# ProteusMRIgHIFU/BabelBrain

Measured on AMD Instinct MI355X. Metric: Mvoxel-steps/sec, 512^3 skull FDTD per device (achieved HBM GB/s in roofline), higher is better.
Workload: dtype f32

## Files before the change

babelbrain_amd/csrc/bfd_api.hip:

```cpp
#include "bfd_internal.h"

#include <math.h>
#include <stdio.h>
#include <string.h>

#include <algorithm>
#include <array>
#include <thread>
#include <hipcub/hipcub.hpp>

static thread_local std::string g_err;
void bfd_set_error(const std::string &s) { g_err = s; }

namespace {

struct HostTables {
    std::vector<float> t;
    float c1, k2;
    double cmax;
};

void fit_sls(double rho, double c, double alpha, double q, double omega, bool exact, double &MR, double &tau)
{
    if (c <= 0.0) { MR = 0.0; tau = 0.0; return; }
// ... 469 lines not shown
        BFD_FAIL(-2, "bfd_create: h, dt, freq must be > 0 and 0 < reflectionLimit < 1");
    int ndev = 0;
    if (hipGetDeviceCount(&ndev) != hipSuccess || ndev <= 0)
        BFD_FAIL(-3, "bfd_create: no HIP device available (this engine has no CPU fallback)");
    if (cfg->device < 0 || cfg->device >= ndev) BFD_FAIL(-3, "bfd_create: device ordinal out of range");
    BFD_HIP(hipSetDevice(cfg->device));

    bfd_sim *s = new bfd_sim();
    s->cfg = *cfg;
    s->step = 0; s->devBytes = 0; s->haveMaterials = s->haveMap = false; s->tilesReady = false;
    s->nSrcVox = 0; s->srcLin = s->srcRow = nullptr; s->srcW[0] = s->srcW[1] = s->srcW[2] = nullptr; s->pulseT = nullptr;
    s->nSources = s->lengthSource = 0;
    s->pulseHost = nullptr; s->tileSteps = s->nTiles = 0;
    s->srcK = 0; s->srcWeights = s->srcSignals = nullptr;
    for (int b = 0; b < 2; b++) { s->tileDev[b] = s->tilePinned[b] = nullptr; s->tileLoaded[b] = s->tilePacked[b] = -1; s->evTile[b] = nullptr; s->evTileUsed[b] = false; for (int q = 0; q < 2; q++) { s->evRead[b][q] = nullptr; s->evReadUsed[b][q] = false; } }
    s->sensEnt = nullptr; s->sensEntValid = false; s->sensIsBox = false; memset(s->sensBox, 0, sizeof s->sensBox);
    s->actBase = nullptr; s->actBytes = 0; s->actReady = false;
    s->nSensors = 0; s->sensLin = nullptr; s->sensOut = nullptr; s->dftAcc = nullptr; s->dftPk = nullptr; s->dftBin = 0;
    s->acc = s->pk = nullptr; s->timing = s->perKernel = false;
    s->pairEnv = true; s->pendingAcc = s->pairDone = false; s->pairedLaunches = 0;
    if (const char *ev = getenv("BFD_PAIR_ACC")) s->pairEnv = atoi(ev) != 0;
    s->advEnv = true; s->midStep = false; s->tiles.advVz = false;
    if (const char *ev = getenv("BFD_ADV_VZ")) s->advEnv = atoi(ev) != 0;
    s->tables = nullptr; s->profiles = nullptr; s->cmax = 0;
    memset(s->algBytes, 0, sizeof s->algBytes); s->tiles.ktimer = nullptr;
    if (hipStreamCreateWithFlags(&s->stream, hipStreamNonBlocking) != hipSuccess) { delete s; BFD_FAIL(-10, "hipStreamCreate failed"); }
    s->ownStream = true;
    if (hipEventCreate(&s->evBegin) != hipSuccess) { hipStreamDestroy(s->stream); delete s; BFD_FAIL(-10, "hipEventCreate failed"); }
    if (hipEventCreate(&s->evEnd) != hipSuccess) { hipEventDestroy(s->evBegin); hipStreamDestroy(s->stream); delete s; BFD_FAIL(-10, "hipEventCreate failed"); }

    bfd_dev &d = s->d;
    memset(&d, 0, sizeof d);
    d.N1 = cfg->N1; d.N2 = cfg->N2; d.N3 = cfg->N3; d.k0 = cfg->k0; d.nk = cfg->nk;
    d.ND = cfg->NDelta; d.P = P; d.plane = cfg->N1 * cfg->N2;
    s->nloc = (size_t)d.plane * d.nk;
    s->nalloc = (size_t)d.plane * (d.nk + 4);
    bfd_placement_cache_evict_other_sizes(cfg->device, s->nalloc * sizeof(float));

    int rc = 0;
    float **fp[15] = {&d.Vx, &d.Vy, &d.Vz, &d.Sxx, &d.Syy, &d.Szz, &d.Sxy, &d.Sxz, &d.Syz,
                      &d.Rxx, &d.Ryy, &d.Rzz, &d.Rxy, &d.Rxz, &d.Ryz};
    for (int a = 0; a < 15 && !rc; a++) {
        rc = dev_alloc(s, &s->stateBase[a], s->nalloc);
        if (!rc) *fp[a] = s->stateBase[a] + 2 * (size_t)d.plane;
    }
    if (!rc) rc = dev_alloc(s, &s->matBase, s->nalloc);
// ... 626 lines not shown
    const bool pairAcc = pair_engine(s, quiet_runs_wanted(s), T.nFluid);
    for (size_t r = 0; r < all.size(); r++) {
        const int4 &run = all[r];
        const int bx = run.x % tx, by = run.x / tx, kb = run.y & 0xFFFF, ke = run.y >> 16, f = run.z;
        const int xa = bx * 64, xb = std::min(xa + 64, N1), ya = by * 8, yb = std::min(ya + 8, N2);
        const double cells = (double)(xb - xa) * (yb - ya) * (ke - kb);
        const double inner = overlap(xa, xb, ND, N1 - ND) * overlap(ya, yb, ND, N2 - ND) * overlap(k0g + kb, k0g + ke, ND, N3 - ND);
        const bool fusedRun = r >= (size_t)(T.nFluid + T.nSolid);
        if (fusedRun) {
            const double fc = 64.0 * bfd_fused_rows() * (ke - kb);
            const double b = 32.0 + ((f & 2) ? 8.0 : 0.0) + ((f & 4) ? 0.0 : 2.0);
            B[0][BFD_K_FUSED] += b * fc; B[1][BFD_K_FUSED] += b * fc + 8.0 * fc;
        } else if (r < (size_t)T.nFluid) {
            const bool lossy = f & 2, uni = f & 4, single = (f & 16) != 0;
            double bs = 12.0 + 8.0 + (lossy ? 8.0 : 0.0) + (uni ? 0.0 : 2.0);
            if (!single) bs += 8.0 + (lossy ? 8.0 : 0.0);
            const double bv = 4.0 + 24.0 + (uni ? 0.0 : 2.0);
            for (int a = 0; a < 2; a++) { B[a][BFD_K_STRESS_FLUID] += bs * cells; B[a][BFD_K_VELOCITY_FLUID] += bv * cells; }
            if (pairAcc) B[1][BFD_K_STRESS_FLUID] += 4.0 * inner; else B[1][BFD_K_VELOCITY_FLUID] += 8.0 * inner;
            if (f & BFD_RUN_ADV_VZ) {
                const double advCells = (double)(xb - xa) * (yb - ya) * std::max(0, ke - kb - 3);
                for (int a = 0; a < 2; a++) { B[a][BFD_K_STRESS_FLUID] += 4.0 * advCells; B[a][BFD_K_VELOCITY_FLUID] -= 8.0 * advCells; }
            }
        } else if (s->cfg.kernelVariant == 2) {
            for (int a = 0; a < 2; a++) { B[a][BFD_K_STRESS_SOLID] += 110.0 * cells; B[a][BFD_K_VELOCITY_SOLID] += 50.0 * cells + (a ? 8.0 * inner : 0.0); }
        } else {
            for (int a = 0; a < 2; a++) B[a][BFD_K_VELOCITY_SOLID] += (a ? 8.0 * inner : 0.0);
        }
    }
    if (T.nSolid && s->cfg.kernelVariant != 2) {
        const double nF0 = (double)cnt[0], nF1 = (double)cnt[1], nS = (double)cnt[2] + (double)cnt[3], nE = (double)cnt[4], nR = (double)cnt[5];
        const double all = nF0 + nF1 + nS + nR;
        const double bs = 15.0 * all + 8.0 * nF0 + 16.0 * nF1 + 48.0 * nS + 48.0 * nR;
        const double bv = 31.0 * all + 8.0 * (nS + nR) + 4.0 * nE;
        const double bsf = 14.0 * all + 8.0 * nF0 + 16.0 * nF1 + 16.0 * nS + 8.0 * nR;
        for (int a = 0; a < 2; a++) { if (s->d.cssRow) B[a][BFD_K_STRESS_FLUID] += bsf; else B[a][BFD_K_STRESS_SOLID] += bs; B[a][BFD_K_VELOCITY_SOLID] += bv; }
    }
    if (s->tiles.nShear) {
        DevTemp<unsigned long long> dc; unsigned long long hc[2] = {0, 0};
        BFD_HIP(dc.alloc(2));
        hipMemsetAsync(dc, 0, sizeof hc, s->stream);
        hipLaunchKernelGGL(count_active_edges, dim3(grid_for(s->tiles.nShear)), dim3(256), 0, s->stream, s->tiles.shearCoef, s->tiles.shearCodes, s->tiles.nShear, dc.p);
        hipMemcpyAsync(hc, dc, sizeof hc, hipMemcpyDeviceToHost, s->stream);
        const hipError_t e = hipStreamSynchronize(s->stream);
        if (e != hipSuccess) BFD_FAIL(-10, std::string("shear edge count: ") + hipGetErrorString(e));
        s->tiles.nShearExplicit = (long)hc[1];
// ... 22 lines not shown
    dev_release(s, &s->tiles.runsAll); s->tiles.nAll = s->tiles.nAllB = 0;
    dev_release(s, &s->tiles.runs); dev_release(s, &s->tiles.xmap); dev_release(s, &s->tiles.shearCells); dev_release(s, &s->tiles.shearCoef); dev_release(s, &s->tiles.shearR);
    dev_release(s, &s->tiles.shearCodes); dev_release(s, &s->tiles.shearTab);
    const TileGrid G = choose_tile_grid(s);
    std::vector<int> flags(G.n, 1), mats(G.n, 0);
    if (s->cfg.kernelVariant != 2) { const int rc = fetch_tile_classes(s, G.n, flags, mats); if (rc) return rc; }
    bfd_tiles &T = s->tiles;
    T.nMat = s->cfg.nMat;
    T.nFluid = T.nFluidB = T.nSolid = T.nSolidB = T.nSolidBP = T.nSolidIP = T.nFused = T.nLossless = T.nLossy = T.nSolidSub = T.nUni = T.nPml = T.nLean = T.nFusedSub = 0;
    s->d.tilesX = G.tx; s->d.tilesY = G.ty;
    if (s->cfg.kernelVariant != 2) for (int id = 0; id < G.n; id++) if (!(flags[id] & 1)) flags[id] |= 16;
    std::vector<int4> lists[5];
    std::vector<int4> listsAll[2];
    std::vector<char> taken((size_t)G.n, 0);
    form_fused_runs(s, G, flags, mats, taken, lists[4]);
    form_two_kernel_runs(s, G, flags, mats, taken, lists, listsAll);
    T.nFluidB = (int)lists[0].size(); T.nFluid = T.nFluidB + (int)lists[1].size();
    T.nSolidB = (int)lists[2].size(); T.nSolid = T.nSolidB + (int)lists[3].size();
    T.nFused = (int)lists[4].size();
    T.advVz = false;
    if (adv_vz_engine(s, T.nSolid))
        for (int a = 0; a < 2; a++)
            for (int4 &run : lists[a])
                if (!(run.z & (1 | 8)) && (run.y >> 16) - (run.y & 0xFFFF) >= 4) { run.z |= BFD_RUN_ADV_VZ; T.advVz = true; }
    std::vector<int4> all;
    for (int a = 0; a < 5; a++) all.insert(all.end(), lists[a].begin(), lists[a].end());
    int rc = dev_alloc(s, &s->tiles.runs, all.size(), false);
    if (rc) return rc;
    BFD_HIP(hipMemcpy(s->tiles.runs, all.data(), all.size() * sizeof(int4), hipMemcpyHostToDevice));
    rc = build_balance_maps(s, all);
    if (rc) return rc;
    s->tiles.nShearExplicit = 0;
    s->tiles.nShear = s->tiles.shearLowEnd = s->tiles.shearHighBeg = 0;
    if (T.nSolid && s->cfg.kernelVariant != 2) {
        int count = 0; bool compact = false; std::vector<unsigned> hostCells;
        rc = build_shear_list(s, G, &count, &compact, hostCells);
        if (!rc && compact) rc = setup_compact_state(s, G, count, listsAll);
        if (!rc && carryCompact) rc = carry_compact_in(s, count, oldCells, oldN, oldComp);
        if (!rc && compact && s->step > 0 && !carryCompact) {
            float *comp[10] = {s->d.cSxx, s->d.cSyy, s->d.cSxy, s->d.cSxz, s->d.cSyz, s->d.cRxx, s->d.cRyy, s->d.cRxy, s->d.cRxz, s->d.cRyz};
            for (int a = 0; a < 10; a++) BFD_HIP(hipMemsetAsync(comp[a], 0, (size_t)count * sizeof(float), s->stream));
            BFD_HIP(hipStreamSynchronize(s->stream));
        }
        if (rc) return rc;
        s->tiles.shearLowEnd = std::lower_bound(hostCells.begin(), hostCells.end(), (unsigned)G.lowPlanes * (unsigned)s->d.plane) - hostCells.begin();
        s->tiles.shearHighBeg = std::lower_bound(hostCells.begin(), hostCells.end(), (unsigned)G.hiStart * (unsigned)s->d.plane) - hostCells.begin();
    } else if (carryCompact) {
// ... 480 lines not shown
```

babelbrain_amd/csrc/bfd_internal.h:

```cpp
#pragma once
#include <hip/hip_runtime.h>
#include <stdint.h>
#include <algorithm>
#include <future>
#include <string>
#include <vector>
#include "../../include/babelfdtd.h"

#define BFD_REFLECTOR_BIT 0x8000u
#define BFD_MAT_MASK 0x7FFFu
#define BFD_CLS_FLUID 1u
#define BFD_CLS_NOMEM 2u
#define BFD_CLS_EXY 4u
#define BFD_CLS_EXZ 8u
#define BFD_CLS_EYZ 16u
#define BFD_CLS_REFL 32u

#ifndef BFD_CA
#define BFD_CA 1.125f
#define BFD_CB (1.0f / 24.0f)
#endif
#ifndef BFD_STAB
#define BFD_STAB (6.0 / 7.0)
#endif
// ... 24 lines not shown
    int actLo, actHi;
};
#define BFD_CSS_NONE 0xFFFFFFFFu
static __device__ __forceinline__ bool css_listed(unsigned c) { return (c & (BFD_CLS_FLUID | BFD_CLS_REFL)) == 0u; }
static __device__ __forceinline__ unsigned css_rank(bool listed)
{
    const unsigned long long b = __ballot(listed);
    return __builtin_amdgcn_mbcnt_hi((unsigned)(b >> 32), __builtin_amdgcn_mbcnt_lo((unsigned)b, 0u));
}
static __device__ __forceinline__ long css_index(const bfd_dev &d, long c)
{
    if (!css_listed(d.cls[c])) return -1;
    const int kl = (int)(c / d.plane);
    const int r = (int)(c - (long)kl * d.plane);
    const int j = r / d.N1, i = r - j * d.N1;
    const unsigned rb = d.cssRow[((long)(kl + 2) * d.N2 + j) * d.cssStride + (i >> 6)];
    if (rb == BFD_CSS_NONE) return -1;
    unsigned n = 0;
    for (long q = c - (i & 63); q < c; q++) n += css_listed(d.cls[q]) ? 1u : 0u;
    return (long)rb + n;
}

#define BFD_RUN_ADV_VZ 512
enum { BFD_K_STRESS_FLUID = 0, BFD_K_STRESS_SOLID = 1, BFD_K_STRESS_SHEAR = 2, BFD_K_VELOCITY_FLUID = 3, BFD_K_VELOCITY_SOLID = 4,
       BFD_K_FUSED = 5, BFD_K_COUNT = 6 };
struct bfd_sim;
void bfd_kmark(bfd_sim *sim, int cls, int end, hipStream_t st);

enum { BFD_XM_SF = 0, BFD_XM_VF = 3, BFD_XM_SS = 6, BFD_XM_VS = 9, BFD_XM_VSP_LO = 12, BFD_XM_VSP_HI = 13, BFD_XM_FUSED = 14, BFD_XMAP_COUNT = 15 };
struct bfd_tiles { bfd_sim *ktimer; int nMat; int4 *runs;
                   unsigned *shearCells; float *shearCoef; long nShear, shearLowEnd, shearHighBeg;
                   unsigned *shearCodes; float *shearTab; long nShearExplicit;
                   int4 *runsAll; int nAll, nAllB;
                   unsigned *cssRow; float *css; long cssCap; bool cssHosted;
                   float *shearR;
                   int nFluid, nFluidB, nSolid, nSolidB, nSolidBP , nSolidIP , nFused ;
                   int nLossless, nLossy, nSolidSub, nUni, nPml, nLean, nFusedSub;
                   bool advVz;
                   int *xmap; int xmapH[BFD_XMAP_COUNT][10]; };

struct bfd_sim {
    bfd_config cfg;
    bfd_dev d;
    hipStream_t stream;
    bool ownStream;
    int step;
// ... 11 lines not shown
    int64_t devBytes;
    bool haveMaterials, haveMap;
    bfd_tiles tiles; bool tilesReady;
    bool pingpong;
    float *ppBase[5];
    int zchunk;
    double cmax;
    int64_t nSrcVox, srcLowEnd, srcHighBeg;
    uint32_t *srcLin, *srcRow; float *srcW[3]; float *pulseT; int nSources, lengthSource;
    const double *pulseHost; int tileSteps, nTiles;
    float *tileDev[2], *tilePinned[2]; int tileLoaded[2], tilePacked[2];
    hipEvent_t evTile[2]; bool evTileUsed[2];
    hipEvent_t evRead[2][2]; bool evReadUsed[2][2];
    std::future<void> packJob[2];
    int srcK; float *srcWeights, *srcSignals;
    unsigned char *actBase; size_t actBytes; bool actReady;
    bool sensIsBox; int sensBox[5];
    int *sensEnt; bool sensEntValid;
    int64_t nSensors; uint32_t *sensLin; float *sensOut; int nTs; int nSelS; int selS[BFD_MAP_COUNT];
    double *dftAcc; float *dftPk; int dftBin;
    int nSelR; int selR[BFD_MAP_COUNT]; float *acc, *pk;
    int accStart;
    bool pairEnv, pendingAcc, pairDone; int64_t pairedLaunches;
    bool advEnv, midStep;
    bool timing, perKernel;
    hipEvent_t evBegin, evEnd;
    std::vector<hipEvent_t> evStress, evVelocity;
    std::vector<hipEvent_t> evK[BFD_K_COUNT];
    double algBytes[2][BFD_K_COUNT];
    std::vector<hipEvent_t> evPool;
    int *stepDev;
    hipGraphExec_t stepGraph;
    hipStream_t captureStream;
    int graphState;
    bool stepDevValid;
};
#define BFD_GRAPH_STEPS 8

void bfd_set_error(const std::string &s);
#define BFD_HIP(call)                                                                              \
    do {                                                                                           \
        hipError_t e_ = (call);                                                                    \
        if (e_ != hipSuccess) {                                                                    \
            bfd_set_error(std::string(#call) + ": " + hipGetErrorString(e_));                      \
            return -10;                                                                            \
        }                                                                                          \
    } while (0)
// ... 85 lines not shown
```

babelbrain_amd/csrc/bfd_kernels_v2.hip:

```cpp
#include "bfd_internal.h"
#include "bfd_device.h"
#include <algorithm>
#include <type_traits>

namespace {

constexpr int TX = BFD_TILE_X;
constexpr int TY = BFD_TILE_Y;
constexpr int LW = TX + 4;
constexpr int LH = TY + 4;
constexpr int NTHREADS = TX * TY;
constexpr int YT = 4 * TX;
constexpr int XT = 4 * TY;
constexpr int ZCHUNK = 32;
constexpr int SUBZ = BFD_SUBZ;
constexpr int STRESS_WAVES_PER_SIMD = 4;
constexpr int FLUID_WAVES_PER_SIMD = 8;
constexpr int VELOCITY_WAVES_PER_SIMD = 4;
constexpr int VELOCITY_FLUID_WAVES_PER_SIMD = FLUID_WAVES_PER_SIMD;

struct HaloTask {
    int lofs;
    int gofs;
    int arr;
// ... 396 lines not shown
__device__ __forceinline__ bool run_all_quiet(const bfd_dev &d, int bx, int by, int kbeg, int kend)
{
    const int q0 = kbeg / SUBZ, q1 = (kend - 1) / SUBZ;
    const int nq = q1 - q0 + 3;
    if (9 * nq > 64) return false;
    if (kbeg < d.actLo || kend > d.actHi) return false;
    const int l = threadIdx.x;
    const int dq = l / 9, r = l - 9 * dq, dy = r / 3, dx = r - 3 * dy;
    const unsigned idx = (unsigned)(((q0 + dq) * d.actY + (by + dy)) * d.actX + (bx + dx));
    const unsigned f = (l < 9 * nq) ? (unsigned)d.act[idx] : 0u;
    return __syncthreads_or(f != 0u) == 0;
}
__device__ __forceinline__ void run_mark_active(const bfd_dev &d, int bx, int by, int kbeg, int kend, unsigned nzbits)
{
    if (__ballot((nzbits & 0x7fffffffu) != 0u) == 0ull) return;
    if (threadIdx.x == 0)
        for (int q = kbeg / SUBZ; q <= (kend - 1) / SUBZ; q++) d.act[((q + 1) * d.actY + by + 1) * d.actX + bx + 1] = 1;
}
__device__ __forceinline__ unsigned fbits(float v) { return __float_as_uint(v); }

template <bool LOSSY, bool COLLAPSED, bool UNI, bool PML, bool SOLID = false, bool QUIET = false, bool PAIR = false>
__device__ __forceinline__ void stress_fluid_body(const bfd_dev &d, int bx, int by, int kbeg, int kend, int tm,
                                                  float (*sV)[2][LH * LW], float *__restrict__ accP = nullptr, float *__restrict__ pkP = nullptr,
                                                  bool advVz = false)
{
    constexpr bool ADVZ = !PML && !SOLID && !QUIET;
    static_assert(!PAIR || (!SOLID && !QUIET), "paired accumulation: plain fluid flavours only");
    unsigned nzb = 0u;
    const int N1 = d.N1, N2 = d.N2;
    const int tx = threadIdx.x, ty = threadIdx.y, tid = ty * TX + tx;
    const int i0 = bx * TX, j0 = by * TY;
    const int i = i0 + tx, j = j0 + ty;
    const bool valid = (i < N1) && (j < N2);
    const long pl = d.plane;
    const int P = d.P;
    const int own = (ty + 2) * LW + tx + 2;
    const unsigned cij = valid ? (unsigned)(j * N1 + i) : 0u;

    HaloTask t; t.lofs = -1; t.ok = false; t.arr = 0; t.gofs = 0;
    if (tid < YT) ytask(tid, 1, i0, j0, N1, N2, t);
    else if (tid < YT + XT) xtask(tid - YT, 0, i0, j0, N1, N2, t);
    const bool has = t.lofs >= 0;
    const float *ph = __builtin_amdgcn_readfirstlane(t.arr) == 0 ? d.Vx : d.Vy;
    const unsigned hofs = t.ok ? (unsigned)t.gofs * 4u : 0u;
    float *lh = &sV[0][t.arr][has ? t.lofs : 0];

    const float c1 = d.c1;
// ... 9 lines not shown
        if (zi) { ax = d.axI[i]; bxc = d.bxI[i]; qx = (unsigned)((kbeg * N2 + j) * (2 * P) + (i < P ? i : i - (N1 - 2 * P))); px = F4(d.psi[0], (unsigned)(qx) * 4u); }
        if (zj) { ay = d.ayI[j]; byc = d.byI[j]; qy = (unsigned)((kbeg * (2 * P) + (j < P ? j : j - (N2 - 2 * P))) * N1 + i); py = F4(d.psi[1], (unsigned)(qy) * 4u); }
        const int kg = d.k0 + kbeg;
        if (valid && (kg < P || kg >= d.N3 - P)) pz = F4(d.psi[2], (unsigned)((long)(kg < P ? kg : kg - (d.N3 - 2 * P)) * pl + cij) * 4u);
    }

    const bool inner = PAIR && valid && i >= d.ND && i < N1 - d.ND && j >= d.ND && j < N2 - d.ND;
    const bool accA = PAIR && accP != nullptr, accK = PAIR && pkP != nullptr;
    float vx0 = 0, vy0 = 0, vzm2 = 0, vzm1 = 0, vz0 = 0, vzp1 = 0, szz = 0, rzz = 0, av = 0;
    unsigned mraw = 0;
    if (valid) {
        const float *bVz = d.Vz + kbeg * pl;
        if (accA) av = LD4((accP + kbeg * pl), cij * 4u);
        vx0 = F4((d.Vx + kbeg * pl), cij * 4u); vy0 = F4((d.Vy + kbeg * pl), cij * 4u);
        vzm2 = LD4((bVz - 2 * pl), cij * 4u); vzm1 = LD4((bVz - pl), cij * 4u); vz0 = LD4(bVz, cij * 4u); vzp1 = LD4((bVz + pl), cij * 4u);
        szz = LD4((d.Szz + kbeg * pl), cij * 4u);
        if (LOSSY) rzz = LD4((d.Rzz + kbeg * pl), cij * 4u);
        if (!UNI) mraw = U2((d.mat + kbeg * pl), cij * 2u);
    }
    float hv = t.ok ? F4(ph + kbeg * pl, hofs) : 0.0f;
    float sq1 = 0, sq2 = 0, sq3 = 0, ruv = 0;
    unsigned mq1 = 0, mq2 = 0;
    if (ADVZ && UNI) ruv = d.invRho[tm];

    for (int kl = kbeg; kl < kend; kl++) {
        const int b = kl & 1;
        const long ko = (long)kl * pl;
        const int k = d.k0 + kl;
        sV[b][0][own] = vx0; sV[b][1][own] = vy0;
        if (has) lh[b * (2 * LH * LW)] = hv;
        float AP = APu, BP = BPu, AS2 = 0.f, BS2 = 0.f;
        if (!UNI && valid) { const int m = mraw & BFD_MAT_MASK; AP = d.AP[m]; if (LOSSY) BP = d.BP[m]; if (SOLID) { AS2 = d.AS2[m]; BS2 = d.BS2[m]; } }
        __syncthreads();

        float nvx = 0, nvy = 0, nvz = 0, nh = 0, nszz = 0, nrzz = 0, npx = 0, npy = 0, npz = 0, nav = 0, nsq = 0;
        unsigned nmraw = 0;
        if (kl + 1 < kend) {
            if (valid) {
                nvx = F4((d.Vx + ko + pl), cij * 4u); nvy = F4((d.Vy + ko + pl), cij * 4u); nvz = LD4((d.Vz + ko + 2 * pl), cij * 4u);
                nszz = LD4((d.Szz + ko + pl), cij * 4u);
                if (accA) nav = LD4((accP + ko + pl), cij * 4u);
                if (LOSSY) nrzz = LD4((d.Rzz + ko + pl), cij * 4u);
                if (!UNI) nmraw = U2((d.mat + ko + pl), cij * 2u);
            }
            if (t.ok) nh = F4(ph + ko + pl, hofs);
            if (PML) {
                if (zi) npx = F4(d.psi[0], (unsigned)(qx + dqx) * 4u);
                if (zj) npy = F4(d.psi[1], (unsigned)(qy + dqy) * 4u);
                const int kn = k + 1;
                if (valid && (kn < P || kn >= d.N3 - P)) npz = F4(d.psi[2], (unsigned)((long)(kn < P ? kn : kn - (d.N3 - 2 * P)) * pl + cij) * 4u);
            }
        }
        if (valid) {
            const float *sx = &sV[b][0][own], *sy = &sV[b][1][own];
            float dxVx = dminus4(sx[-2], sx[-1], vx0, sx[1]);
            float dyVy = dminus4(sy[-2 * LW], sy[-LW], vy0, sy[LW]);
// ... 34 lines not shown
                        if (an > m) m = an;
                        if (m > m0) F4((pkP + ko), cij * 4u) = m;
                    }
                }
            }
            if (QUIET) nzb |= fbits(val) | fbits(rn);
            if (!COLLAPSED) { F4((d.Sxx + ko), cij * 4u) = val; F4((d.Syy + ko), cij * 4u) = val; }
            if (LOSSY) {
                ST4((d.RzzW + ko), cij * 4u, rn);
                if (!COLLAPSED) { F4((d.Rxx + ko), cij * 4u) = rn; F4((d.Ryy + ko), cij * 4u) = rn; }
            }
            if (ADVZ) {
                nsq = val;
                if (advVz && kl >= kbeg + 3) {
                    float r0 = ruv, r1 = ruv;
                    if (!UNI) { r0 = d.invRho[mq2 & BFD_MAT_MASK]; r1 = d.invRho[mq1 & BFD_MAT_MASK]; }
                    const float dz = dplus4(sq3, sq2, sq1, val);
                    float w = vzm2 + (0.5f * (r0 + r1)) * dz;
                    if (!UNI && (mq2 & BFD_REFLECTOR_BIT)) w = 0.f;
                    ST4((d.VzW + ko - 2 * pl), cij * 4u, w);
                }
            }
        }
        if (ADVZ) { sq3 = sq2; sq2 = sq1; sq1 = nsq; mq2 = mq1; mq1 = mraw; }
        vx0 = nvx; vy0 = nvy;
        vzm2 = vzm1; vzm1 = vz0; vz0 = vzp1; vzp1 = nvz;
        hv = nh; szz = nszz; rzz = nrzz; mraw = nmraw; av = nav;
        px = npx; py = npy; pz = npz; qx += dqx; qy += dqy;
    }
    if (QUIET) run_mark_active(d, bx, by, kbeg, kend, nzb);
}

template <bool ACC, bool UNI, bool PML, bool QUIET = false>
__device__ __forceinline__ void velocity_fluid_body(const bfd_dev &d, int bx, int by, int kbeg, int kend, int tm,
                                                    float (*sS)[LH * LW], float *__restrict__ accP, float *__restrict__ pkP, bool advVz = false)
{
    const bool adv = !PML && !QUIET && advVz;
    const int N1 = d.N1, N2 = d.N2;
    const int tx = threadIdx.x, ty = threadIdx.y, tid = ty * TX + tx;
    const int i0 = bx * TX, j0 = by * TY;
    const int i = i0 + tx, j = j0 + ty;
    const bool valid = (i < N1) && (j < N2);
    const long pl = d.plane;
    const int P = d.P;
    const int own = (ty + 2) * LW + tx + 2;
    const unsigned cij = valid ? (unsigned)(j * N1 + i) : 0u;
    const unsigned cx = valid ? (unsigned)(j * N1 + min(i + 1, N1 - 1)) : 0u;
    const unsigned cy = valid ? (unsigned)(min(j + 1, N2 - 1) * N1 + i) : 0u;

    HaloTask t; t.lofs = -1; t.ok = false; t.arr = 0; t.gofs = 0;
    if (tid < YT) ytask(tid, 0, i0, j0, N1, N2, t);
    else if (tid < YT + XT) xtask(tid - YT, 0, i0, j0, N1, N2, t);
    const bool has = t.lofs >= 0;
    const float *ph = d.Szz;
    const unsigned hofs = t.ok ? (unsigned)t.gofs * 4u : 0u;
    float *lh = &sS[0][has ? t.lofs : 0];

    const bool inner = valid && i >= d.ND && i < N1 - d.ND && j >= d.ND && j < N2 - d.ND;
    const bool accA = ACC && accP != nullptr, accK = ACC && pkP != nullptr;
    unsigned nzb = 0u;
    float ru = 0.f;
    if (UNI) ru = d.invRho[tm];

    const bool zi = PML && valid && (i < P || i >= N1 - P);
    const bool zj = PML && valid && (j < P || j >= N2 - P);
    float ax = 0, bxc = 0, ay = 0, byc = 0, px = 0, py = 0, pz = 0;
    unsigned qx = 0, qy = 0;
    const unsigned dqx = (unsigned)(N2 * 2 * P), dqy = (unsigned)(2 * P * N1);
    if (PML) {
        if (zi) { ax = d.axH[i]; bxc = d.bxH[i]; qx = (unsigned)((kbeg * N2 + j) * (2 * P) + (i < P ? i : i - (N1 - 2 * P))); px = F4(d.psi[9], (unsigned)(qx) * 4u); }
        if (zj) { ay = d.ayH[j]; byc = d.byH[j]; qy = (unsigned)((kbeg * (2 * P) + (j < P ? j : j - (N2 - 2 * P))) * N1 + i); py = F4(d.psi[13], (unsigned)(qy) * 4u); }
        const int kg = d.k0 + kbeg;
        if (valid && (kg < P || kg >= d.N3 - P)) pz = F4(d.psi[17], (unsigned)((long)(kg < P ? kg : kg - (d.N3 - 2 * P)) * pl + cij) * 4u);
    }

    float sm1 = 0, s0 = 0, sp1 = 0, sp2 = 0, vx = 0, vy = 0, vz = 0, av = 0, r0 = ru;
    unsigned mraw = 0, mraw1 = 0, mx = 0, my = 0;
    if (valid) {
        const float *bS = d.Szz + kbeg * pl;
        sm1 = F4((bS - pl), cij * 4u); s0 = F4(bS, cij * 4u); sp1 = F4((bS + pl), cij * 4u); sp2 = F4((bS + 2 * pl), cij * 4u);
        vx = LD4((d.Vx + kbeg * pl), cij * 4u); vy = LD4((d.Vy + kbeg * pl), cij * 4u); vz = LD4((d.Vz + kbeg * pl), cij * 4u);
        if (accA) av = LD4((accP + kbeg * pl), cij * 4u);
        if (!UNI) {
            const uint16_t *bM = d.mat + kbeg * pl;
            mraw = U2(bM, cij * 2u); mraw1 = U2((bM + pl), cij * 2u); mx = U2(bM, cx * 2u); my = U2(bM, cy * 2u);
            r0 = d.invRho[mraw & BFD_MAT_MASK];
        }
    }
    float hv = t.ok ? F4(ph + kbeg * pl, hofs) : 0.0f;

    for (int kl = kbeg; kl < kend; kl++) {
        const int b = kl & 1;
        const long ko = (long)kl * pl;
        const int k = d.k0 + kl;
        sS[b][own] = s0;
        if (has) lh[b * (LH * LW)] = hv;
        float r1 = ru, rx = ru, ry = ru;
        if (!UNI && valid) {
            r1 = d.invRho[mraw1 & BFD_MAT_MASK];
            rx = d.invRho[mx & BFD_MAT_MASK];
            ry = d.invRho[my & BFD_MAT_MASK];
        }
        __syncthreads();

        float ns = 0, nh = 0, nvx = 0, nvy = 0, nvz = 0, nav = 0, npx = 0, npy = 0, npz = 0;
        unsigned nm2 = 0, nmx = 0, nmy = 0;
        if (!UNI && valid) nm2 = U2((d.mat + ko + 2 * pl), cij * 2u);
        if (kl + 1 < kend) {
            if (valid) {
                ns = F4((d.Szz + ko + 3 * pl), cij * 4u);
                nvx = LD4((d.Vx + ko + pl), cij * 4u); nvy = LD4((d.Vy + ko + pl), cij * 4u);
                if (!(adv && kl + 1 < kend - 2)) nvz = LD4((d.Vz + ko + pl), cij * 4u);
                if (!UNI) { nmx = U2((d.mat + ko + pl), cx * 2u); nmy = U2((d.mat + ko + pl), cy * 2u); }
                if (accA) nav = LD4((accP + ko + pl), cij * 4u);
            }
            if (t.ok) nh = F4(ph + ko + pl, hofs);
            if (PML) {
                if (zi) npx = F4(d.psi[9], (unsigned)(qx + dqx) * 4u);
                if (zj) npy = F4(d.psi[13], (unsigned)(qy + dqy) * 4u);
                const int kn = k + 1;
                if (valid && (kn < P || kn >= d.N3 - P)) npz = F4(d.psi[17], (unsigned)((long)(kn < P ? kn : kn - (d.N3 - 2 * P)) * pl + cij) * 4u);
            }
        }
        const bool ownVz = !(adv && kl > kbeg && kl < kend - 2);
        if (valid) {
            if (ACC) {
                if (inner && k >= d.ND && k < d.N3 - d.ND) {
                    const float s = (s0 + s0) + s0;
                    const float p = -s * (1.0f / 3.0f);
                    if (accA) ST4((accP + ko), cij * 4u, av + p * p);
                    if (accK) { const float ap = fabsf(p); if (ap > F4((pkP + ko), cij * 4u)) F4((pkP + ko), cij * 4u) = ap; }
                }
            }
            if (!UNI && (mraw & BFD_REFLECTOR_BIT)) {
                F4((d.VxW + ko), cij * 4u) = 0.f; F4((d.VyW + ko), cij * 4u) = 0.f;
                if (ownVz) F4((d.VzW + ko), cij * 4u) = 0.f;
            } else {
                const float *p = &sS[b][own];
                float dx = dplus4(p[-1], s0, p[1], p[2]);
                float dy = dplus4(p[-LW], s0, p[LW], p[2 * LW]);
                float dz = dplus4(sm1, s0, sp1, sp2);
                if (PML) {
                    if (zi) { const float pn = bxc * px + ax * dx; F4(d.psi[9], (unsigned)(qx) * 4u) = pn; dx = dx + pn; }
                    if (zj) { const float pn = byc * py + ay * dy; F4(d.psi[13], (unsigned)(qy) * 4u) = pn; dy = dy + pn; }
                    if (k < P || k >= d.N3 - P) {
                        const float pn = d.bzH[k] * pz + d.azH[k] * dz;
                        F4(d.psi[17], (unsigned)((long)(k < P ? k : k - (d.N3 - 2 * P)) * pl + cij) * 4u) = pn;
                        dz = dz + pn;
                    }
                }
                if (!QUIET) {
                    ST4((d.VxW + ko), cij * 4u, vx + (0.5f * (r0 + rx)) * dx);
                    ST4((d.VyW + ko), cij * 4u, vy + (0.5f * (r0 + ry)) * dy);
                    if (ownVz) ST4((d.VzW + ko), cij * 4u, vz + (0.5f * (r0 + r1)) * dz);
                } else {
                    { const float w = vx + (0.5f * (r0 + rx)) * dx; ST4((d.VxW + ko), cij * 4u, w); nzb |= fbits(w); }
                    { const float w = vy + (0.5f * (r0 + ry)) * dy; ST4((d.VyW + ko), cij * 4u, w); nzb |= fbits(w); }
                    { const float w = vz + (0.5f * (r0 + r1)) * dz; ST4((d.VzW + ko), cij * 4u, w); nzb |= fbits(w); }
                }
            }
        }
        sm1 = s0; s0 = sp1; sp1 = sp2; sp2 = ns;
        hv = nh; vx = nvx; vy = nvy; vz = nvz; av = nav;
        r0 = r1; mraw = mraw1; mraw1 = nm2; mx = nmx; my = nmy;
        px = npx; py = npy; pz = npz; qx += dqx; qy += dqy;
    }
    if (QUIET) run_mark_active(d, bx, by, kbeg, kend, nzb);
}

template <bool PML>
__device__ __forceinline__ void stress_solid_body(const bfd_dev &d, const int4 &run, int tilesX, float (*sV)[2][LH * LW])
{
    const int N1 = d.N1, N2 = d.N2;
    const int bx = run.x % tilesX, by = run.x / tilesX, kbeg = run.y & 0xFFFF, kend = run.y >> 16;
    const int tx = threadIdx.x, ty = threadIdx.y, tid = ty * TX + tx;
    const int i0 = bx * TX, j0 = by * TY;
// ... 739 lines not shown
    for (int q = 0; q < 6; q++) coef[6 * t + q] = o[q];
    if (codes) {
        auto code = [&](float A, int ma, int mb, int mc) { return A == 0.f ? 0u : ((m == ma && m == mb && m == mc && m < 254) ? (unsigned)(1 + m) : 255u); };
        codes[t] = code(o[0], mx, my, mxy) | (code(o[2], mx, mz, mxz) << 8) | (code(o[4], my, mz, myz) << 16) | (m < 255 ? (unsigned)(1 + m) << 24 : 0u);
    }
}
__global__ void shear_material_table(bfd_dev d, float *__restrict__ tab, int nMat)
{
    const int m = blockIdx.x * blockDim.x + threadIdx.x;
    if (m >= nMat) return;
    const float iv0 = d.invMu[m], t0 = d.tauS[m], k2 = d.k2;
    float A = 0.f, B = 0.f;
    if (iv0 > 0.f) {
        const float muH = 4.0f / ((iv0 + iv0) + (iv0 + iv0));
        const float tau = 0.25f * ((t0 + t0) + (t0 + t0));
        A = muH * (1.0f + tau); B = (muH * tau) * k2;
    }
    tab[8 * m] = A; tab[8 * m + 1] = B; tab[8 * m + 2] = 0.f; tab[8 * m + 3] = 0.f;
    tab[8 * m + 4] = d.AP[m]; tab[8 * m + 5] = d.BP[m]; tab[8 * m + 6] = d.AS2[m]; tab[8 * m + 7] = d.BS2[m];
}

template <bool COLLAPSED, bool QUIET = false, bool PAIR = false>
__device__ __forceinline__ void stress_fluid_switch(const bfd_dev &d, const int4 &run, int tilesX, float (*sV)[2][LH * LW],
                                                    float *__restrict__ accP = nullptr, float *__restrict__ pkP = nullptr)
{
    const int bx = run.x % tilesX, by = run.x / tilesX, kbeg = run.y & 0xFFFF, kend = run.y >> 16, tm = run.w;
    const bool adv = (run.z & BFD_RUN_ADV_VZ) != 0;
    if (QUIET && run_all_quiet(d, bx, by, kbeg, kend)) return;
    if (run.z & 1) {
        if (run.z & 8) stress_fluid_body<true, true, false, true, true, QUIET>(d, bx, by, kbeg, kend, tm, sV);
        else stress_fluid_body<true, true, false, false, true, QUIET>(d, bx, by, kbeg, kend, tm, sV);
        return;
    }
    switch ((run.z >> 1) & 7) {
    case 0: stress_fluid_body<false, COLLAPSED, false, false, false, QUIET, PAIR>(d, bx, by, kbeg, kend, tm, sV, accP, pkP, adv); break;
    case 1: stress_fluid_body<true, COLLAPSED, false, false, false, QUIET, PAIR>(d, bx, by, kbeg, kend, tm, sV, accP, pkP, adv); break;
    case 2: stress_fluid_body<false, COLLAPSED, true, false, false, QUIET, PAIR>(d, bx, by, kbeg, kend, tm, sV, accP, pkP, adv); break;
    case 3: stress_fluid_body<true, COLLAPSED, true, false, false, QUIET, PAIR>(d, bx, by, kbeg, kend, tm, sV, accP, pkP, adv); break;
    case 4: stress_fluid_body<false, COLLAPSED, false, true, false, QUIET, PAIR>(d, bx, by, kbeg, kend, tm, sV, accP, pkP); break;
    case 5: stress_fluid_body<true, COLLAPSED, false, true, false, QUIET, PAIR>(d, bx, by, kbeg, kend, tm, sV, accP, pkP); break;
    case 6: stress_fluid_body<false, COLLAPSED, true, true, false, QUIET, PAIR>(d, bx, by, kbeg, kend, tm, sV, accP, pkP); break;
    default: stress_fluid_body<true, COLLAPSED, true, true, false, QUIET, PAIR>(d, bx, by, kbeg, kend, tm, sV, accP, pkP); break;
    }
}

template <bool COLLAPSED, bool QUIET = false, bool PAIR = false>
__global__ __launch_bounds__(NTHREADS, FLUID_WAVES_PER_SIMD) void stress_fluid(bfd_dev d, int tilesX, int nblocks, const int *__restrict__ xmap,
                                                                               const int4 *__restrict__ runs,
                                                                               float *__restrict__ accP, float *__restrict__ pkP)
{
    __shared__ float sV[2][2][LH * LW];
    const int ri = run_index(nblocks, xmap);
    if (ri < 0) return;
    const int4 run = runs[ri];
    if (COLLAPSED || (run.z & 16)) stress_fluid_switch<true, QUIET, PAIR>(d, run, tilesX, sV, accP, pkP);
    else stress_fluid_switch<false, QUIET, PAIR>(d, run, tilesX, sV, accP, pkP);
}

__global__ __launch_bounds__(NTHREADS) void flush_paired_pressure(bfd_dev d, int tilesX, int nruns, const int4 *__restrict__ runs,
                                                                  float *__restrict__ accP, float *__restrict__ pkP)
{
    if ((int)blockIdx.x >= nruns) return;
    const int4 run = runs[blockIdx.x];
    const int bx = run.x % tilesX, by = run.x / tilesX, kbeg = run.y & 0xFFFF, kend = run.y >> 16;
    const int i = bx * TX + (int)threadIdx.x, j = by * TY + (int)threadIdx.y;
    if (!(i >= d.ND && i < d.N1 - d.ND && j >= d.ND && j < d.N2 - d.ND)) return;
    const long cij = (long)j * d.N1 + i;
    for (int kl = kbeg; kl < kend; kl++) {
        const int k = d.k0 + kl;
        if (k < d.ND || k >= d.N3 - d.ND) continue;
        const long c = (long)kl * d.plane + cij;
        const float s0 = d.Szz[c];
        const float s = (s0 + s0) + s0;
        const float p = -s * (1.0f / 3.0f);
        if (accP) accP[c] = accP[c] + p * p;
        if (pkP) { const float ap = fabsf(p); if (ap > pkP[c]) pkP[c] = ap; }
    }
}

template <bool ACC, bool QUIET = false>
__global__ __launch_bounds__(NTHREADS, VELOCITY_FLUID_WAVES_PER_SIMD) void velocity_fluid(bfd_dev d, int tilesX, int nblocks, const int *__restrict__ xmap,
                                                                                 const int4 *__restrict__ runs,
                                                                                 float *__restrict__ accP, float *__restrict__ pkP)
{
    __shared__ float sS[2][LH * LW];
    const int ri = run_index(nblocks, xmap);
    if (ri < 0) return;
    const int4 run = runs[ri];
    const int bx = run.x % tilesX, by = run.x / tilesX, kbeg = run.y & 0xFFFF, kend = run.y >> 16, tm = run.w;
    const bool adv = (run.z & BFD_RUN_ADV_VZ) != 0;
    if (QUIET && run_all_quiet(d, bx, by, kbeg, kend)) return;
    switch ((run.z >> 2) & 3) {
    case 0: velocity_fluid_body<ACC, false, false, QUIET>(d, bx, by, kbeg, kend, tm, sS, accP, pkP, adv); break;
    case 1: velocity_fluid_body<ACC, true, false, QUIET>(d, bx, by, kbeg, kend, tm, sS, accP, pkP, adv); break;
    case 2: velocity_fluid_body<ACC, false, true, QUIET>(d, bx, by, kbeg, kend, tm, sS, accP, pkP); break;
    default: velocity_fluid_body<ACC, true, true, QUIET>(d, bx, by, kbeg, kend, tm, sS, accP, pkP); break;
    }
}

__global__ void classify_tiles(bfd_dev d, int tilesX, int tilesY, int *__restrict__ flags, int *__restrict__ tileMat)
{
    const int tile = blockIdx.x;
    const int bx = tile % tilesX, by = (tile / tilesX) % tilesY, bz = tile / (tilesX * tilesY);
    const int i0 = bx * TX - 2, j0 = by * TY - 2, k0 = bz * SUBZ - 2;
    const int nzOwn = min(SUBZ, d.nk - bz * SUBZ);
    const int nx = TX + 4, ny = TY + 4, nz = nzOwn + 4;
    const unsigned first = d.mat[(long)(bz * SUBZ) * d.plane + (long)min(by * TY, d.N2 - 1) * d.N1 + min(bx * TX, d.N1 - 1)];
    int solid = 0, lossy = 0, lossyG = 0, refl = 0, mixed = (first & BFD_REFLECTOR_BIT) ? 1 : 0;
    for (int v = threadIdx.x; v < nx * ny * nz; v += blockDim.x) {
        const int li = v % nx, lj = (v / nx) % ny, lk = v / (nx * ny);
        const int i = i0 + li, j = j0 + lj, kl = k0 + lk;
        if (i < 0 || i >= d.N1 || j < 0 || j >= d.N2) continue;
        const unsigned raw = d.mat[(long)kl * d.plane + (long)j * d.N1 + i];
        const int m = raw & BFD_MAT_MASK;
        if (raw != first) mixed = 1;
        if (raw & BFD_REFLECTOR_BIT) refl = 1;
        if (d.invMu[m] > 0.f) solid = 1;
// ... 265 lines not shown
```

Measured before the change: 97320.

## Advance interior Vy rows inside the fluid stress kernel to skip velocity reloads

Extends the existing advance-Vz scheme to the y velocity component. For interior tile rows, the fluid stress kernel now computes and stores the Vy update from freshly computed stress values, staged in new shared buffers (sN, sR). The fluid velocity kernel then skips loading, updating and storing Vy and the y-neighbour material for those rows. The aim is to cut HBM traffic in this bandwidth-bound stencil. In exchange it adds shared memory, extra barriers and extra work per stress block, which may lower occupancy.

Result: no change. 98140 (median of 6 runs) (+0.8%).

```diff
diff --git a/babelbrain_amd/csrc/bfd_api.hip b/babelbrain_amd/csrc/bfd_api.hip
--- a/babelbrain_amd/csrc/bfd_api.hip
+++ b/babelbrain_amd/csrc/bfd_api.hip
@@ -515,6 +515,8 @@
     if (const char *ev = getenv("BFD_PAIR_ACC")) s->pairEnv = atoi(ev) != 0;
     s->advEnv = true; s->midStep = false; s->tiles.advVz = false;
     if (const char *ev = getenv("BFD_ADV_VZ")) s->advEnv = atoi(ev) != 0;
+    s->advYEnv = true;
+    if (const char *ev = getenv("BFD_ADV_VY")) s->advYEnv = atoi(ev) != 0;
     s->tables = nullptr; s->profiles = nullptr; s->cmax = 0;
     memset(s->algBytes, 0, sizeof s->algBytes); s->tiles.ktimer = nullptr;
     if (hipStreamCreateWithFlags(&s->stream, hipStreamNonBlocking) != hipSuccess) { delete s; BFD_FAIL(-10, "hipStreamCreate failed"); }
@@ -1187,6 +1189,10 @@
                 const double advCells = (double)(xb - xa) * (yb - ya) * std::max(0, ke - kb - 3);
                 for (int a = 0; a < 2; a++) { B[a][BFD_K_STRESS_FLUID] += 4.0 * advCells; B[a][BFD_K_VELOCITY_FLUID] -= 8.0 * advCells; }
             }
+            if (f & BFD_RUN_ADV_VY) {
+                const double advCells = (double)(xb - xa) * std::max(0, std::min(yb, ya + 6) - (ya + 1)) * (ke - kb);
+                for (int a = 0; a < 2; a++) { B[a][BFD_K_STRESS_FLUID] += 4.0 * advCells; B[a][BFD_K_VELOCITY_FLUID] -= 8.0 * advCells; }
+            }
         } else if (s->cfg.kernelVariant == 2) {
             for (int a = 0; a < 2; a++) { B[a][BFD_K_STRESS_SOLID] += 110.0 * cells; B[a][BFD_K_VELOCITY_SOLID] += 50.0 * cells + (a ? 8.0 * inner : 0.0); }
         } else {
@@ -1255,7 +1261,11 @@
     if (adv_vz_engine(s, T.nSolid))
         for (int a = 0; a < 2; a++)
             for (int4 &run : lists[a])
-                if (!(run.z & (1 | 8)) && (run.y >> 16) - (run.y & 0xFFFF) >= 4) { run.z |= BFD_RUN_ADV_VZ; T.advVz = true; }
+                if (!(run.z & (1 | 8))) {
+                    const int planes = (run.y >> 16) - (run.y & 0xFFFF);
+                    if (planes >= 4) { run.z |= BFD_RUN_ADV_VZ; T.advVz = true; }
+                    if (s->advYEnv && s->d.VyW == s->d.Vy && planes >= 1) { run.z |= BFD_RUN_ADV_VY; T.advVz = true; }
+                }
     std::vector<int4> all;
     for (int a = 0; a < 5; a++) all.insert(all.end(), lists[a].begin(), lists[a].end());
     int rc = dev_alloc(s, &s->tiles.runs, all.size(), false);
diff --git a/babelbrain_amd/csrc/bfd_internal.h b/babelbrain_amd/csrc/bfd_internal.h
--- a/babelbrain_amd/csrc/bfd_internal.h
+++ b/babelbrain_amd/csrc/bfd_internal.h
@@ -70,6 +70,7 @@
 }
 
 #define BFD_RUN_ADV_VZ 512
+#define BFD_RUN_ADV_VY 1024
 enum { BFD_K_STRESS_FLUID = 0, BFD_K_STRESS_SOLID = 1, BFD_K_STRESS_SHEAR = 2, BFD_K_VELOCITY_FLUID = 3, BFD_K_VELOCITY_SOLID = 4,
        BFD_K_FUSED = 5, BFD_K_COUNT = 6 };
 struct bfd_sim;
@@ -127,7 +128,7 @@
     int nSelR; int selR[BFD_MAP_COUNT]; float *acc, *pk;
     int accStart;
     bool pairEnv, pendingAcc, pairDone; int64_t pairedLaunches;
-    bool advEnv, midStep;
+    bool advEnv, advYEnv, midStep;
     bool timing, perKernel;
     hipEvent_t evBegin, evEnd;
     std::vector<hipEvent_t> evStress, evVelocity;
diff --git a/babelbrain_amd/csrc/bfd_kernels_v2.hip b/babelbrain_amd/csrc/bfd_kernels_v2.hip
--- a/babelbrain_amd/csrc/bfd_kernels_v2.hip
+++ b/babelbrain_amd/csrc/bfd_kernels_v2.hip
@@ -442,7 +442,7 @@
 template <bool LOSSY, bool COLLAPSED, bool UNI, bool PML, bool SOLID = false, bool QUIET = false, bool PAIR = false>
 __device__ __forceinline__ void stress_fluid_body(const bfd_dev &d, int bx, int by, int kbeg, int kend, int tm,
                                                   float (*sV)[2][LH * LW], float *__restrict__ accP = nullptr, float *__restrict__ pkP = nullptr,
-                                                  bool advVz = false)
+                                                  bool advVz = false, bool advVy = false, float (*sN)[TY * TX] = nullptr, float (*sR)[TY * TX] = nullptr)
 {
     constexpr bool ADVZ = !PML && !SOLID && !QUIET;
     static_assert(!PAIR || (!SOLID && !QUIET), "paired accumulation: plain fluid flavours only");
@@ -498,6 +498,18 @@
     float sq1 = 0, sq2 = 0, sq3 = 0, ruv = 0;
     unsigned mq1 = 0, mq2 = 0;
     if (ADVZ && UNI) ruv = d.invRho[tm];
+    const bool rowVy = ADVZ && advVy && ty >= 1 && ty <= TY - 3 && valid;
+    const bool upIn = j + 1 < N2;
+    auto storeVy = [&](int p, float sOwn, unsigned idOwn) {
+        const int pb = p & 1;
+        const float *q = &sN[pb][tid];
+        float r0 = ruv, ry = ruv;
+        if (!UNI) { r0 = sR[pb][tid]; ry = upIn ? sR[pb][tid + TX] : r0; }
+        const float dy = dplus4(q[-TX], sOwn, q[TX], q[2 * TX]);
+        float w = sV[pb][1][own] + (0.5f * (r0 + ry)) * dy;
+        if (!UNI && (idOwn & BFD_REFLECTOR_BIT)) w = 0.f;
+        ST4((d.VyW + (long)p * pl), cij * 4u, w);
+    };
 
     for (int kl = kbeg; kl < kend; kl++) {
         const int b = kl & 1;
@@ -506,8 +518,10 @@
         sV[b][0][own] = vx0; sV[b][1][own] = vy0;
         if (has) lh[b * (2 * LH * LW)] = hv;
         float AP = APu, BP = BPu, AS2 = 0.f, BS2 = 0.f;
-        if (!UNI && valid) { const int m = mraw & BFD_MAT_MASK; AP = d.AP[m]; if (LOSSY) BP = d.BP[m]; if (SOLID) { AS2 = d.AS2[m]; BS2 = d.BS2[m]; } }
+        float rown = 0.f;
+        if (!UNI && valid) { const int m = mraw & BFD_MAT_MASK; AP = d.AP[m]; if (LOSSY) BP = d.BP[m]; if (SOLID) { AS2 = d.AS2[m]; BS2 = d.BS2[m]; } if (ADVZ && advVy) rown = d.invRho[m]; }
         __syncthreads();
+        if (ADVZ && rowVy && kl > kbeg) storeVy(kl - 1, sq1, mq1);
 
         float nvx = 0, nvy = 0, nvz = 0, nh = 0, nszz = 0, nrzz = 0, npx = 0, npy = 0, npz = 0, nav = 0, nsq = 0;
         unsigned nmraw = 0;
@@ -588,20 +602,27 @@
                 }
             }
         }
+        if (ADVZ && advVy) { sN[b][tid] = nsq; if (!UNI) sR[b][tid] = rown; }
         if (ADVZ) { sq3 = sq2; sq2 = sq1; sq1 = nsq; mq2 = mq1; mq1 = mraw; }
         vx0 = nvx; vy0 = nvy;
         vzm2 = vzm1; vzm1 = vz0; vz0 = vzp1; vzp1 = nvz;
         hv = nh; szz = nszz; rzz = nrzz; mraw = nmraw; av = nav;
         px = npx; py = npy; pz = npz; qx += dqx; qy += dqy;
     }
+    if (ADVZ && advVy) {
+        __syncthreads();
+        if (rowVy) storeVy(kend - 1, sq1, mq1);
+    }
     if (QUIET) run_mark_active(d, bx, by, kbeg, kend, nzb);
 }
 
 template <bool ACC, bool UNI, bool PML, bool QUIET = false>
 __device__ __forceinline__ void velocity_fluid_body(const bfd_dev &d, int bx, int by, int kbeg, int kend, int tm,
-                                                    float (*sS)[LH * LW], float *__restrict__ accP, float *__restrict__ pkP, bool advVz = false)
+                                                    float (*sS)[LH * LW], float *__restrict__ accP, float *__restrict__ pkP, bool advVz = false,
+                                                    bool advVy = false)
 {
     const bool adv = !PML && !QUIET && advVz;
+    const bool ownVy = !(!PML && !QUIET && advVy && threadIdx.y >= 1 && threadIdx.y <= TY - 3);
     const int N1 = d.N1, N2 = d.N2;
     const int tx = threadIdx.x, ty = threadIdx.y, tid = ty * TX + tx;
     const int i0 = bx * TX, j0 = by * TY;
@@ -645,11 +666,11 @@
     if (valid) {
         const float *bS = d.Szz + kbeg * pl;
         sm1 = F4((bS - pl), cij * 4u); s0 = F4(bS, cij * 4u); sp1 = F4((bS + pl), cij * 4u); sp2 = F4((bS + 2 * pl), cij * 4u);
-        vx = LD4((d.Vx + kbeg * pl), cij * 4u); vy = LD4((d.Vy + kbeg * pl), cij * 4u); vz = LD4((d.Vz + kbeg * pl), cij * 4u);
+        vx = LD4((d.Vx + kbeg * pl), cij * 4u); if (ownVy) vy = LD4((d.Vy + kbeg * pl), cij * 4u); vz = LD4((d.Vz + kbeg * pl), cij * 4u);
         if (accA) av = LD4((accP + kbeg * pl), cij * 4u);
         if (!UNI) {
             const uint16_t *bM = d.mat + kbeg * pl;
-            mraw = U2(bM, cij * 2u); mraw1 = U2((bM + pl), cij * 2u); mx = U2(bM, cx * 2u); my = U2(bM, cy * 2u);
+            mraw = U2(bM, cij * 2u); mraw1 = U2((bM + pl), cij * 2u); mx = U2(bM, cx * 2u); if (ownVy) my = U2(bM, cy * 2u);
             r0 = d.invRho[mraw & BFD_MAT_MASK];
         }
     }
@@ -665,7 +686,7 @@
         if (!UNI && valid) {
             r1 = d.invRho[mraw1 & BFD_MAT_MASK];
             rx = d.invRho[mx & BFD_MAT_MASK];
-            ry = d.invRho[my & BFD_MAT_MASK];
+            if (ownVy) ry = d.invRho[my & BFD_MAT_MASK];
         }
         __syncthreads();
 
@@ -675,9 +696,9 @@
         if (kl + 1 < kend) {
             if (valid) {
                 ns = F4((d.Szz + ko + 3 * pl), cij * 4u);
-                nvx = LD4((d.Vx + ko + pl), cij * 4u); nvy = LD4((d.Vy + ko + pl), cij * 4u);
+                nvx = LD4((d.Vx + ko + pl), cij * 4u); if (ownVy) nvy = LD4((d.Vy + ko + pl), cij * 4u);
                 if (!(adv && kl + 1 < kend - 2)) nvz = LD4((d.Vz + ko + pl), cij * 4u);
-                if (!UNI) { nmx = U2((d.mat + ko + pl), cx * 2u); nmy = U2((d.mat + ko + pl), cy * 2u); }
+                if (!UNI) { nmx = U2((d.mat + ko + pl), cx * 2u); if (ownVy) nmy = U2((d.mat + ko + pl), cy * 2u); }
                 if (accA) nav = LD4((accP + ko + pl), cij * 4u);
             }
             if (t.ok) nh = F4(ph + ko + pl, hofs);
@@ -699,7 +720,7 @@
                 }
             }
             if (!UNI && (mraw & BFD_REFLECTOR_BIT)) {
-                F4((d.VxW + ko), cij * 4u) = 0.f; F4((d.VyW + ko), cij * 4u) = 0.f;
+                F4((d.VxW + ko), cij * 4u) = 0.f; if (ownVy) F4((d.VyW + ko), cij * 4u) = 0.f;
                 if (ownVz) F4((d.VzW + ko), cij * 4u) = 0.f;
             } else {
                 const float *p = &sS[b][own];
@@ -717,7 +738,7 @@
                 }
                 if (!QUIET) {
                     ST4((d.VxW + ko), cij * 4u, vx + (0.5f * (r0 + rx)) * dx);
-                    ST4((d.VyW + ko), cij * 4u, vy + (0.5f * (r0 + ry)) * dy);
+                    if (ownVy) ST4((d.VyW + ko), cij * 4u, vy + (0.5f * (r0 + ry)) * dy);
                     if (ownVz) ST4((d.VzW + ko), cij * 4u, vz + (0.5f * (r0 + r1)) * dz);
                 } else {
                     { const float w = vx + (0.5f * (r0 + rx)) * dx; ST4((d.VxW + ko), cij * 4u, w); nzb |= fbits(w); }
@@ -1503,10 +1524,11 @@
 
 template <bool COLLAPSED, bool QUIET = false, bool PAIR = false>
 __device__ __forceinline__ void stress_fluid_switch(const bfd_dev &d, const int4 &run, int tilesX, float (*sV)[2][LH * LW],
+                                                    float (*sN)[TY * TX], float (*sR)[TY * TX],
                                                     float *__restrict__ accP = nullptr, float *__restrict__ pkP = nullptr)
 {
     const int bx = run.x % tilesX, by = run.x / tilesX, kbeg = run.y & 0xFFFF, kend = run.y >> 16, tm = run.w;
-    const bool adv = (run.z & BFD_RUN_ADV_VZ) != 0;
+    const bool adv = (run.z & BFD_RUN_ADV_VZ) != 0, advY = (run.z & BFD_RUN_ADV_VY) != 0;
     if (QUIET && run_all_quiet(d, bx, by, kbeg, kend)) return;
     if (run.z & 1) {
         if (run.z & 8) stress_fluid_body<true, true, false, true, true, QUIET>(d, bx, by, kbeg, kend, tm, sV);
@@ -1514,10 +1536,10 @@
         return;
     }
     switch ((run.z >> 1) & 7) {
-    case 0: stress_fluid_body<false, COLLAPSED, false, false, false, QUIET, PAIR>(d, bx, by, kbeg, kend, tm, sV, accP, pkP, adv); break;
-    case 1: stress_fluid_body<true, COLLAPSED, false, false, false, QUIET, PAIR>(d, bx, by, kbeg, kend, tm, sV, accP, pkP, adv); break;
-    case 2: stress_fluid_body<false, COLLAPSED, true, false, false, QUIET, PAIR>(d, bx, by, kbeg, kend, tm, sV, accP, pkP, adv); break;
-    case 3: stress_fluid_body<true, COLLAPSED, true, false, false, QUIET, PAIR>(d, bx, by, kbeg, kend, tm, sV, accP, pkP, adv); break;
+    case 0: stress_fluid_body<false, COLLAPSED, false, false, false, QUIET, PAIR>(d, bx, by, kbeg, kend, tm, sV, accP, pkP, adv, advY, sN, sR); break;
+    case 1: stress_fluid_body<true, COLLAPSED, false, false, false, QUIET, PAIR>(d, bx, by, kbeg, kend, tm, sV, accP, pkP, adv, advY, sN, sR); break;
+    case 2: stress_fluid_body<false, COLLAPSED, true, false, false, QUIET, PAIR>(d, bx, by, kbeg, kend, tm, sV, accP, pkP, adv, advY, sN, sR); break;
+    case 3: stress_fluid_body<true, COLLAPSED, true, false, false, QUIET, PAIR>(d, bx, by, kbeg, kend, tm, sV, accP, pkP, adv, advY, sN, sR); break;
     case 4: stress_fluid_body<false, COLLAPSED, false, true, false, QUIET, PAIR>(d, bx, by, kbeg, kend, tm, sV, accP, pkP); break;
     case 5: stress_fluid_body<true, COLLAPSED, false, true, false, QUIET, PAIR>(d, bx, by, kbeg, kend, tm, sV, accP, pkP); break;
     case 6: stress_fluid_body<false, COLLAPSED, true, true, false, QUIET, PAIR>(d, bx, by, kbeg, kend, tm, sV, accP, pkP); break;
@@ -1531,11 +1553,12 @@
                                                                                float *__restrict__ accP, float *__restrict__ pkP)
 {
     __shared__ float sV[2][2][LH * LW];
+    __shared__ float sN[2][TY * TX], sR[2][TY * TX];
     const int ri = run_index(nblocks, xmap);
     if (ri < 0) return;
     const int4 run = runs[ri];
-    if (COLLAPSED || (run.z & 16)) stress_fluid_switch<true, QUIET, PAIR>(d, run, tilesX, sV, accP, pkP);
-    else stress_fluid_switch<false, QUIET, PAIR>(d, run, tilesX, sV, accP, pkP);
+    if (COLLAPSED || (run.z & 16)) stress_fluid_switch<true, QUIET, PAIR>(d, run, tilesX, sV, sN, sR, accP, pkP);
+    else stress_fluid_switch<false, QUIET, PAIR>(d, run, tilesX, sV, sN, sR, accP, pkP);
 }
 
 __global__ __launch_bounds__(NTHREADS) void flush_paired_pressure(bfd_dev d, int tilesX, int nruns, const int4 *__restrict__ runs,
@@ -1569,11 +1592,11 @@
     if (ri < 0) return;
     const int4 run = runs[ri];
     const int bx = run.x % tilesX, by = run.x / tilesX, kbeg = run.y & 0xFFFF, kend = run.y >> 16, tm = run.w;
-    const bool adv = (run.z & BFD_RUN_ADV_VZ) != 0;
+    const bool adv = (run.z & BFD_RUN_ADV_VZ) != 0, advY = (run.z & BFD_RUN_ADV_VY) != 0;
     if (QUIET && run_all_quiet(d, bx, by, kbeg, kend)) return;
     switch ((run.z >> 2) & 3) {
-    case 0: velocity_fluid_body<ACC, false, false, QUIET>(d, bx, by, kbeg, kend, tm, sS, accP, pkP, adv); break;
-    case 1: velocity_fluid_body<ACC, true, false, QUIET>(d, bx, by, kbeg, kend, tm, sS, accP, pkP, adv); break;
+    case 0: velocity_fluid_body<ACC, false, false, QUIET>(d, bx, by, kbeg, kend, tm, sS, accP, pkP, adv, advY); break;
+    case 1: velocity_fluid_body<ACC, true, false, QUIET>(d, bx, by, kbeg, kend, tm, sS, accP, pkP, adv, advY); break;
     case 2: velocity_fluid_body<ACC, false, true, QUIET>(d, bx, by, kbeg, kend, tm, sS, accP, pkP); break;
     default: velocity_fluid_body<ACC, true, true, QUIET>(d, bx, by, kbeg, kend, tm, sS, accP, pkP); break;
     }
```
